# OpenDriveLab/OccNet

Hardware: NVIDIA H100
Metric: samples/s (6-cam->200x200x16 voxel) (higher is better)
Workload: dtype bf16

## Files before the change

include/occ_b200.h:

```cpp
#ifndef OCC_B200_H_
#define OCC_B200_H_

#include <stdint.h>

#ifdef __cplusplus
extern "C" {
#endif

const char* occb200_last_error(void);
const char* occb200_version(void);

int occb200_ms_deform_attn_forward(const float* value, const int64_t* spatial_shapes,
                                   const int64_t* level_start_index, const float* sampling_loc,
                                   const float* attn_weight, int B, int Nv, int M, int C, int Nq, int L, int P,
                                   int im2col_step, float* out, void* stream);

int occb200_ms_deform_attn_backward(const float* value, const int64_t* spatial_shapes, const int64_t* level_start_index,
                                    const float* sampling_loc, const float* attn_weight, const float* grad_output, int B,
                                    int Nv, int M, int C, int Nq, int L, int P, int im2col_step, float* grad_value,
                                    float* grad_sampling_loc, float* grad_attn_weight, void* stream);

typedef struct occb200_engine occb200_engine;
typedef struct occb200_backbone occb200_backbone;

// ... 46 lines not shown
int occb200_engine_forward_video(occb200_engine* e, const float* const* feats, const int32_t* rot_map_dev, int scene_start,
                                 float* bev_embed, float* occ_logits, float* flow, uint8_t* occ_cls_u8, int64_t* occ_cls_i64,
                                 void* stream);
int occb200_engine_submit_host_video(occb200_engine* e, int slot, const float* const* feats_host, const int32_t* rot_map_host,
                                     int scene_start, int64_t* occ_cls_i64_host, float* flow_host, void* stream);
int occb200_engine_forward_video_angle(occb200_engine* e, const float* const* feats, double angle_deg, int scene_start,
                                       float* bev_embed, float* occ_logits, float* flow, uint8_t* occ_cls_u8,
                                       int64_t* occ_cls_i64, void* stream);
int occb200_engine_submit_host_video_angle(occb200_engine* e, int slot, const float* const* feats_host, double angle_deg,
                                           int scene_start, int64_t* occ_cls_i64_host, float* flow_host, void* stream);

int occb200_engine_enable_taps(occb200_engine* e, int enable);
int occb200_engine_copy_tap(occb200_engine* e, int which, int layer, float* dst_dev, void* stream);

int occb200_engine_project_pillars(occb200_engine* e, float* ref_cam, uint8_t* mask, void* stream);
int occb200_engine_launches_per_frame(const occb200_engine* e);
int occb200_engine_profile(occb200_engine* e, int enable);
int occb200_engine_profile_read(occb200_engine* e, float* ms_per_category, int* launches_per_category, int n);

int occb200_render_forward(const float* sigma, const float* origin, const float* points, const float* tindex,
                           int N, int T, int Z, int Y, int X, int64_t M, float* pred_dist, float* gt_dist,
                           float* coord_index, void* stream);

int occb200_ray_metric_accumulate(const uint8_t* sem_pred, const float* flow_pred, const uint8_t* sem_gt,
                                  const float* flow_gt, const void* origins, int origin_is_f64, int T,
                                  const float* rays, int M, double* counters, float* pcd_pred, float* pcd_gt,
                                  void* stream);

int occb200_linear_f32(const float* A, const float* W, const float* bias, const float* residual, float* C, int M,
                       int N, int K, int act, void* stream);
// ... 36 lines not shown
```

occnet_b200/_lib.py:

```python
import ctypes
import os

_HERE = os.path.dirname(os.path.abspath(__file__))
LIB_PATH = os.path.join(_HERE, 'lib', 'libocc_b200.so')

c_f32p = ctypes.c_void_p
_vp = ctypes.c_void_p
_i = ctypes.c_int
_i64 = ctypes.c_int64
_f64 = ctypes.c_double


class OccConfig(ctypes.Structure):
    _fields_ = [('bev_h', _i), ('bev_w', _i), ('embed_dims', _i), ('num_heads', _i), ('num_layers', _i),
                ('num_cams', _i), ('num_levels', _i), ('level_h', _i * 4), ('level_w', _i * 4),
                ('num_points_in_pillar', _i), ('sca_points', _i), ('tsa_points', _i), ('ffn_dim', _i),
                ('pillar_h', _i), ('out_dim', _i), ('num_classes', _i), ('pc_range', ctypes.c_float * 6),
                ('precision', _i), ('use_tensor_cores', _i), ('use_cams_embeds', _i),
                ('rotate_center', _i * 2)]


SIGNATURES = {
    'occb200_last_error': (ctypes.c_char_p, []),
    'occb200_version': (ctypes.c_char_p, []),
# ... 10 lines not shown
    'occb200_engine_set_prev_rotation_angle': (_i, [_vp, _f64]),
    'occb200_rotation_coeffs': (_i, [_f64, _i, _i, _i, _i, _vp]),
    'occb200_engine_rotation_map': (_i, [_vp, _f64, _vp, _vp]),
    'occb200_engine_forward': (_i, [_vp, ctypes.POINTER(_vp), _vp, _vp, _vp, _vp, _vp, _vp, _vp]),
    'occb200_engine_forward_host': (_i, [_vp, ctypes.POINTER(_vp), _vp, _vp, _vp]),
    'occb200_engine_submit_host': (_i, [_vp, _i, ctypes.POINTER(_vp), _vp, _vp, _vp]),
    'occb200_engine_wait_host': (_i, [_vp, _i]),
    'occb200_engine_set_history': (_i, [_vp, _i]),
    'occb200_engine_forward_video': (_i, [_vp, ctypes.POINTER(_vp), _vp, _i, _vp, _vp, _vp, _vp, _vp, _vp]),
    'occb200_engine_submit_host_video': (_i, [_vp, _i, ctypes.POINTER(_vp), _vp, _i, _vp, _vp, _vp]),
    'occb200_engine_forward_video_angle': (_i, [_vp, ctypes.POINTER(_vp), _f64, _i, _vp, _vp, _vp, _vp, _vp, _vp]),
    'occb200_engine_submit_host_video_angle': (_i, [_vp, _i, ctypes.POINTER(_vp), _f64, _i, _vp, _vp, _vp]),
    'occb200_engine_enable_taps': (_i, [_vp, _i]),
    'occb200_engine_copy_tap': (_i, [_vp, _i, _i, _vp, _vp]),
    'occb200_engine_project_pillars': (_i, [_vp, _vp, _vp, _vp]),
    'occb200_engine_launches_per_frame': (_i, [_vp]),
    'occb200_engine_profile': (_i, [_vp, _i]),
    'occb200_engine_profile_read': (_i, [_vp, _vp, _vp, _i]),
    'occb200_render_forward': (_i, [_vp, _vp, _vp, _vp, _i, _i, _i, _i, _i, _i64, _vp, _vp, _vp, _vp]),
    'occb200_ray_metric_accumulate': (_i, [_vp, _vp, _vp, _vp, _vp, _i, _i, _vp, _i, _vp, _vp, _vp, _vp]),
    'occb200_linear_f32': (_i, [_vp, _vp, _vp, _vp, _vp, _i, _i, _i, _i, _vp]),
    'occb200_layernorm_f32': (_i, [_vp, _vp, _vp, _vp, _i, _i, _vp]),
    'occb200_gemm_bf16_tc': (_i, [_vp, _vp, _vp, _vp, _i, _i, _i, _vp]),
    'occb200_gemm_tc': (_i, [_vp, _vp, _i, _vp, _vp, _vp, _vp, _i, _i, _i, _i, _i, _vp]),
    'occb200_gemm_tc_ln': (_i, [_vp, _vp, _vp, _vp, _vp, _vp, _vp, _vp, _vp, _vp, _i, _i, _vp]),
    'occb200_gemm_tc_blocked256': (_i, [_vp, _vp, _vp, _vp, _i, _i, _i, _vp]),
    'occb200_gemm_tc_tsa_inputs': (_i, [_vp, _i, _vp, _vp, _vp, _vp, _vp, _i, _vp, _vp, _vp, _vp, _vp, _i, _i, _i, _vp]),
    'occb200_gemm_tc_split3': (_i, [_vp, _i, _vp, _vp, _vp, _vp, _i, _i, _i, _vp]),
    'occb200_split_bf16': (_i, [_vp, _i, _vp, _i, _i64, _vp, _vp]),
    'occb200_backbone_create': (_vp, [_i, _i, _i, _i, _i]),
# ... 49 lines not shown
```

occnet_b200/csrc/engine.cu:

```cuda
#include <cuda_runtime.h>

#include <algorithm>
#include <cmath>
#include <cstring>
#include <map>
#include <string>
#include <vector>

#include "../../include/occ_b200.h"
#include "common.cuh"
#include "conv3d_tc.cuh"
#include "gemm_tc.cuh"
#include "kernels.cuh"

namespace occ {

static thread_local std::string g_last_error;
void set_last_error(const std::string& msg) { g_last_error = msg; }

namespace {

struct DevBuf {
    void* p = nullptr;
    size_t bytes = 0;
// ... 16 lines not shown
    DevBuf tsa_v_wh, tsa_q_wh, tsa_o_wh, sca_q_wh, sca_v_wh, sca_o_wh, ffn1_wh, ffn2_wh;
    DevBuf tsa_q_wh_fold, tsa_q_const, tsa_q_const_t32;
};

}
}

using namespace occ;

struct occb200_engine {
    occb200_config cfg;
    int Nq = 0, Nv = 0, C = 256;
    LevelGeom lg;
    ScaParams sp;
    bool cameras_set = false, finalized = false, taps = false;
    DevBuf rot_map;
    bool rot_set = false;
    RotGrid rot_grid;
    bool rot_grid_set = false;
    DevBuf hist;
    bool hist_valid = false;
    cudaEvent_t hist_done = nullptr;
    bool hist_recorded = false;
    int feats_bf16 = 0;
    occb200_backbone* bb = nullptr;
    DevBuf bb_levels[4];
    cudaEvent_t bb_free = nullptr;
    bool bb_free_recorded = false;
    std::map<std::string, std::vector<float>> host_params;
    std::vector<LayerW> layers;
// ... 82 lines not shown
    occb200_engine* e; cudaStream_t st; int cat; cudaEvent_t a = nullptr, b = nullptr;
    static cudaEvent_t get(occb200_engine* e) {
        if (e->event_used == e->event_pool.size()) {
            cudaEvent_t ev; cudaEventCreate(&ev); e->event_pool.push_back(ev);
        }
        return e->event_pool[e->event_used++];
    }
    ProfScope(occb200_engine* e_, cudaStream_t st_, int cat_) : e(e_), st(st_), cat(cat_) {
        if (e->profiling) { a = get(e); b = get(e); cudaEventRecord(a, st); }
    }
    ~ProfScope() {
        if (e->profiling) { cudaEventRecord(b, st); e->prof_events.push_back({cat, {a, b}}); }
    }
};

template <typename TA, typename TC>
int gemm(occb200_engine* e, const TA* A, const TA* A2, int K1, const float* W, const void* Wh, const float* bias,
         const float* residual, TC* C, int M, int N, int K, int act, cudaStream_t st)
{
    e->launches++;
    ProfScope ps(e, st, CAT_GEMM);
    if constexpr (sizeof(TA) == 2) {
        if (e->cfg.use_tensor_cores && Wh != nullptr && gemm_tc_supported(M, N, K, A2 != nullptr ? K1 : K)) {
            return gemm_tc<TC>(reinterpret_cast<const bf16*>(A), reinterpret_cast<const bf16*>(A2), K1,
                               reinterpret_cast<const bf16*>(Wh), bias, residual, C, M, N, K, act, st);
        }
    }
    if constexpr (sizeof(TA) == 4 && std::is_same<TC, float>::value) {
        if (e->cfg.use_tensor_cores && e->cfg.precision == 0 && Wh != nullptr && e->split_ws.p != nullptr &&
            gemm_tc_supported(M, N, 3 * K, 2 * K)) {
// ... 144 lines not shown
    const int nq_sca = 8 * c.num_levels * c.sca_points * 3;
    const bool q_half = sizeof(T) == 2 && c.use_tensor_cores && e->layers[0].tsa_q_wh.p != nullptr &&
                        e->layers[0].sca_q_wh.p != nullptr && gemm_tc_supported(Nq, nq_tsa, 2 * C, C) &&
                        gemm_tc_supported(Nq, nq_sca, C, C);
    void* qproj = e->qproj.p;
    T* attn_out = e->attn_out.as<T>();
    const bool hoist_v = sizeof(T) == 2 && c.use_tensor_cores && e->sca_value_all.p != nullptr;
    const bool l0_fold = mode == MODE_FRAME && const_q && !has_prev && e->l0_ready;
    const T* q_t_in = q_t;
    if (hoist_v && mode == MODE_FRAME) {
        e->launches++;
        ProfScope ps(e, st, CAT_GEMM);
        if (gemm_tc_blocked256((const bf16*)tokens, e->sca_v_all_wh.as<bf16>(), e->sca_v_all_b.as<float>(),
                               e->sca_value_all.as<bf16>(), ncam * Nv, c.num_layers * C, C, st)) return 2;
    }
    for (int l = 0; l < c.num_layers; ++l) {
        LayerW& w = e->layers[l];
        const bool fold_pos = fuse_ln && !has_prev && w.tsa_q_wh_fold.p != nullptr && w.tsa_q_const.p != nullptr && q_half;
        if (l == 0 && l0_fold) {
            q_f32 = e->l0_x_f32.as<float>(); x_f32 = e->q_f32.as<float>(); spare_f32 = e->x_f32.as<float>();
            cbuf = q_f32;
            q_t_in = e->l0_q_t.as<T>();
            q_in = q_t; q_pos_in = q_pos_t;
        } else {
            const T* a_v = has_prev ? e->prev_t.as<T>() : q_in;
            T* v_prev = e->tsa_value.as<T>();
            const T* v_cur = has_prev ? e->tsa_v_query.as<T>() + (size_t)l * Nq * C : v_prev;
            const bool tsa_merge = sizeof(T) == 2 && fuse_ln && q_half && w.tsa_v_wh.p != nullptr;
            if (tsa_merge) {
                if constexpr (sizeof(T) == 2) {
// ... 52 lines not shown
            }
        }
        const int rc = q_half ? gemm<T, __half>(e, q_t_in, nullptr, 0, w.sca_q_w.as<float>(), w.sca_q_wh.p, w.sca_q_b.as<float>(),
                                                nullptr, (__half*)qproj, Nq, nq_sca, C, ACT_NONE, st)
                              : gemm<T, float>(e, q_t_in, nullptr, 0, w.sca_q_w.as<float>(), w.sca_q_wh.p, w.sca_q_b.as<float>(),
                                               nullptr, (float*)qproj, Nq, nq_sca, C, ACT_NONE, st);
        if (rc) return 2;
        q_t_in = q_t;
        const T* sca_val = e->sca_value.as<T>();
        if (hoist_v) {
            sca_val = reinterpret_cast<const T*>(e->sca_value_all.as<bf16>() + (size_t)l * ncam * Nv * C);
        } else if (gemm<T, T>(e, tokens, nullptr, 0, w.sca_v_w.as<float>(), w.sca_v_wh.p, w.sca_v_b.as<float>(), nullptr,
                              e->sca_value.as<T>(), ncam * Nv, C, C, ACT_NONE, st)) return 2;
        {
            ProfScope ps(e, st, CAT_SCA);
            if (launch_sca_fused<T>(sca_val, qproj, q_half, e->sp, e->lg, Nv, attn_out, e->hits.as<uint8_t>(), st)) return 2;
        }
        e->launches++;
        if (fuse_ln) {
            if (gemm_ln_fused(e, (const bf16*)attn_out, w.sca_o_wh.p, w.sca_o_b.as<float>(), q_f32, w.ln_g[1].as<float>(),
                              w.ln_b[1].as<float>(), nullptr, x_f32, (bf16*)q_t, nullptr, Nq, C, st)) return 2;
            advance();
        } else {
            if (gemm<T, float>(e, attn_out, nullptr, 0, w.sca_o_w.as<float>(), w.sca_o_wh.p, w.sca_o_b.as<float>(),
                               q_f32, x_f32, Nq, C, C, ACT_NONE, st)) return 2;
            if (e->taps)
                OCC_CUDA(cudaMemcpyAsync(e->tap_sca.as<float>() + (size_t)l * Nq * C, x_f32, (size_t)Nq * C * 4,
                                         cudaMemcpyDeviceToDevice, st));
            {
                ProfScope ps(e, st, CAT_LN);
                if (launch_layernorm<T>(x_f32, w.ln_g[1].as<float>(), w.ln_b[1].as<float>(), nullptr, Nq, C, q_f32, q_t,
// ... 12 lines not shown
                return 2;
            advance();
        } else {
            if (gemm<T, float>(e, e->ffn_h.as<T>(), nullptr, 0, w.ffn2_w.as<float>(), w.ffn2_wh.p, w.ffn2_b.as<float>(),
                               q_f32, x_f32, Nq, C, c.ffn_dim, ACT_NONE, st)) return 2;
            {
                ProfScope ps(e, st, CAT_LN);
                if (launch_layernorm<T>(x_f32, w.ln_g[2].as<float>(), w.ln_b[2].as<float>(), pos, Nq, C, q_f32, y_t,
                                        q_pos_t, st)) return 2;
            }
            e->launches++;
        }
        if (e->taps)
            OCC_CUDA(cudaMemcpyAsync(e->tap_layer.as<float>() + (size_t)l * Nq * C, q_f32, (size_t)Nq * C * 4,
                                     cudaMemcpyDeviceToDevice, st));
    }
    const int X = c.bev_w, Y = c.bev_h, Z = c.pillar_h, mid = C / Z;
    const bool lift_from_t32 = fuse_ln && sizeof(T) == 2 && bev_embed == nullptr && Z == 16 && mid == 16;
    if (fuse_ln && !lift_from_t32) {
        ProfScope ps(e, st, CAT_PACK);
        if (launch_t32_convert(q_f32, x_f32, Nq, 1, st)) return 2;
        advance();
        e->launches++;
    }
    if (bev_embed)
        OCC_CUDA(cudaMemcpyAsync(bev_embed, q_f32, (size_t)Nq * C * 4, cudaMemcpyDeviceToDevice, st));
    if (!occ_logits && !flow && !cls_u8 && !cls_i64) return 0;
    {
        ProfScope ps(e, st, CAT_VOX);
        if (lift_from_t32) {
// ... 214 lines not shown
{
    if (!e) return;
    for (auto& w : e->layers) {
        DevBuf* all[] = {&w.tsa_v_w, &w.tsa_v_b, &w.tsa_q_w, &w.tsa_q_b, &w.tsa_o_w, &w.tsa_o_b, &w.sca_q_w, &w.sca_q_b,
                         &w.sca_v_w, &w.sca_v_b, &w.sca_o_w, &w.sca_o_b, &w.ffn1_w, &w.ffn1_b, &w.ffn2_w, &w.ffn2_b,
                         &w.ln_g[0], &w.ln_g[1], &w.ln_g[2], &w.ln_b[0], &w.ln_b[1], &w.ln_b[2], &w.tsa_v_wh,
                         &w.tsa_q_wh, &w.tsa_o_wh, &w.sca_q_wh, &w.sca_v_wh, &w.sca_o_wh, &w.ffn1_wh, &w.ffn2_wh,
                         &w.tsa_q_wh_fold, &w.tsa_q_const, &w.tsa_q_const_t32};
        for (DevBuf* b : all) b->release();
    }
    DevBuf* all[] = {&e->rot_map, &e->hist, &e->split_ws, &e->tokens_split, &e->l0_x_f32, &e->l0_q_t, &e->pos_bf, &e->qc_f32, &e->qc_t, &e->qc_pos_t, &e->bev_queries, &e->pos, &e->pos_t32, &e->cams_embeds, &e->level_embeds, &e->conv_w[0], &e->conv_w[1],
                     &e->conv_b[0], &e->conv_b[1], &e->conv_wh[0], &e->conv_wh[1], &e->conv_wh_hi[0], &e->conv_wh_hi[1], &e->conv_wh_lo[0],
                     &e->conv_wh_lo[1], &e->vox_split, &e->sca_v_all_wh, &e->sca_v_all_b, &e->sca_value_all, &e->hw1, &e->hb1, &e->hw2, &e->hb2,
                     &e->fw1, &e->fb1, &e->fw2, &e->fb2, &e->head_w1h, &e->head_w2h, &e->head_b1c, &e->head_b2c, &e->tokens, &e->sca_value, &e->q_f32, &e->q_t,
                     &e->q_pos_t, &e->prev_t, &e->tsa_value, &e->tsa_v_query, &e->qproj, &e->attn_out,
                     &e->x_f32, &e->ffn_h, &e->vox0, &e->vox1, &e->vox2, &e->hits, &e->tap_layer, &e->tap_tsa,
                     &e->tap_sca, &e->feats_dev[0], &e->feats_dev[1], &e->feats_dev[2], &e->feats_dev[3],
                     &e->occ_i64_dev, &e->flow_dev, &e->bb_levels[0], &e->bb_levels[1], &e->bb_levels[2], &e->bb_levels[3]};
    for (DevBuf* b : all) b->release();
    if (e->bb_free) cudaEventDestroy(e->bb_free);
    if (e->hist_done) cudaEventDestroy(e->hist_done);
    for (auto& sl : e->slots) {
        for (auto& f : sl.feats) f.release();
        sl.occ.release(); sl.flow.release(); sl.rot.release();
        if (sl.rot_pinned) cudaFreeHost(sl.rot_pinned);
        if (sl.compute_done) {
            for (cudaEvent_t ev : sl.h2d_done) cudaEventDestroy(ev);
            cudaEventDestroy(sl.compute_done); cudaEventDestroy(sl.d2h_done);
        }
    }
    if (e->d2h_stream) {
        for (cudaStream_t hs : e->h2d_stream) cudaStreamDestroy(hs);
        cudaStreamDestroy(e->d2h_stream);
    }
    for (cudaEvent_t ev : e->event_pool) cudaEventDestroy(ev);
    delete e;
// ... 203 lines not shown
                upload(e->head_b1c, b1c.data(), b1c.size()) || upload(e->head_b2c, b2c.data(), b2c.size())) return 2;
        }
    }
    const size_t es = e->elt();
    const size_t nvox = (size_t)c.bev_w * c.bev_h * c.pillar_h;
    const size_t ntok = (size_t)c.num_cams * e->Nv;
    int maxq = 8 * c.num_levels * c.sca_points * 3;
    const size_t nq_pad = ((size_t)Nq + 127) / 128 * 128;
    if (e->tokens.alloc(ntok * C * es) || e->sca_value.alloc(ntok * C * es) || e->q_f32.alloc(nq_pad * C * 4) ||
        e->q_t.alloc((size_t)Nq * C * es) || e->q_pos_t.alloc((size_t)Nq * C * es) ||
        e->prev_t.alloc((size_t)Nq * C * es) || e->tsa_value.alloc((size_t)Nq * C * es) ||
        e->qproj.alloc((size_t)Nq * maxq * 4) ||
        e->attn_out.alloc((size_t)Nq * C * es) || e->x_f32.alloc(nq_pad * C * 4) ||
        e->ffn_h.alloc((size_t)Nq * F * es) || e->vox0.alloc(nvox * mid * es) || e->vox1.alloc(nvox * od * es) ||
        e->vox2.alloc(nvox * od * es) || e->hits.alloc(Nq)) return 2;
    OCC_CUDA(cudaMemset(e->q_f32.p, 0, nq_pad * C * 4));
    OCC_CUDA(cudaMemset(e->x_f32.p, 0, nq_pad * C * 4));
    if (tc32) {
        const size_t kmax = (size_t)std::max(2 * C, F);
        if (e->split_ws.alloc((size_t)Nq * 2 * kmax * 2) || e->tokens_split.alloc(ntok * 2 * C * 2)) return 2;
        if (c.pillar_h == 16 && e->vox_split.alloc(nvox * 2 * od * 2)) return 2;
    }
    e->host_params.clear();
    if ((c.precision == 0 ? build_tsa_query_values<float>(e) : build_tsa_query_values<bf16>(e))) return 2;
    e->l0_ready = false;
    if (tc && e->qc_f32.p != nullptr && getenv("OCC_NO_L0_FOLD") == nullptr) {
        const size_t rows_pad = ((size_t)Nq + 127) / 128 * 128;
        if (e->l0_x_f32.alloc(rows_pad * C * 4) || e->l0_q_t.alloc((size_t)Nq * C * 2)) return 2;
        OCC_CUDA(cudaMemset(e->l0_x_f32.p, 0, rows_pad * C * 4));
        const bool taps = e->taps;
        e->taps = false;
        const int rc = forward_impl<bf16>(e, nullptr, nullptr, nullptr, nullptr, nullptr, nullptr, nullptr, 0, MODE_L0_TSA_ONLY);
        e->taps = taps;
        if (rc) return rc;
        OCC_CUDA(cudaDeviceSynchronize());
        e->l0_ready = true;
    }
    e->finalized = true;
    return 0;
}

int occb200_engine_set_cameras(occb200_engine* e, const float* cam_mat, const float* zs, int img_h, int img_w)
{
    OCC_CHECK(e && cam_mat && zs, "null pointer");
    const occb200_config& c = e->cfg;
    memset(&e->sp, 0, sizeof(e->sp));
    for (int i = 0; i < c.num_cams; ++i)
        for (int k = 0; k < 16; ++k) e->sp.cam_mat[i][k] = cam_mat[i * 16 + k];
    for (int i = 0; i < c.num_points_in_pillar; ++i) e->sp.zs[i] = zs[i];
    for (int i = 0; i < 3; ++i) {
        e->sp.pc_scale[i] = (float)((double)c.pc_range[3 + i] - (double)c.pc_range[i]);
        e->sp.pc_min[i] = c.pc_range[i];
    }
    e->sp.img_w = (float)img_w; e->sp.img_h = (float)img_h;
    e->sp.num_cams = c.num_cams; e->sp.D = c.num_points_in_pillar; e->sp.bev_h = c.bev_h; e->sp.bev_w = c.bev_w;
    e->cameras_set = true;
    return 0;
}

int occb200_engine_forward(occb200_engine* e, const float* const* feats, const float* prev_bev, float* bev_embed,
                           float* occ_logits, float* flow, uint8_t* occ_cls_u8, int64_t* occ_cls_i64, void* stream)
{
    OCC_CHECK(e && feats, "null pointer");
    if (check_frame(e, feats)) return 1;
    return run_frame(e, feats, prev_bev, bev_embed, occ_logits, flow, occ_cls_u8, occ_cls_i64, (cudaStream_t)stream);
}

int occb200_engine_set_history(occb200_engine* e, int enable)
{
    OCC_CHECK(e, "null engine");
    if (e->hist_recorded) OCC_CUDA(cudaEventSynchronize(e->hist_done));
    e->hist_recorded = false;
// ... 266 lines not shown
            OCC_CUDA(cudaMemcpyAsync(dst, e->tokens.p, nt * 4, cudaMemcpyDeviceToDevice, st));
            return 0;
        }
        return launch_bf16_to_f32(e->tokens.as<bf16>(), dst, (int64_t)nt, st);
    }
    set_last_error("unknown tap");
    return 1;
}

int occb200_engine_project_pillars(occb200_engine* e, float* ref_cam, uint8_t* mask, void* stream)
{
    OCC_CHECK(e && ref_cam && mask && e->cameras_set, "null pointer / cameras not set");
    return launch_project_pillars(e->sp, ref_cam, mask, (cudaStream_t)stream);
}

int occb200_engine_launches_per_frame(const occb200_engine* e) { return e ? e->launches : 0; }

int occb200_engine_profile(occb200_engine* e, int enable)
{
    OCC_CHECK(e, "null engine");
    e->profiling = enable != 0;
    e->prof_events.clear();
    e->event_used = 0;
    return 0;
}

int occb200_engine_profile_read(occb200_engine* e, float* ms_per_category, int* launches_per_category, int n)
{
    OCC_CHECK(e && ms_per_category && launches_per_category && n >= CAT_COUNT, "bad arguments");
    OCC_CUDA(cudaDeviceSynchronize());
// ... 122 lines not shown
```

occnet_b200/csrc/kernels.cuh:

```cuda
#pragma once
#include "common.cuh"

typedef struct occb200_backbone occb200_backbone;

namespace occ {

struct ScaParams {
    float cam_mat[8][16];
    float zs[8];
    float pc_scale[3];
    float pc_min[3];
    float img_w, img_h;
    int num_cams, D, bev_h, bev_w;
};

int launch_msda_forward(const float* value, const int64_t* shapes, const int64_t* lstart, const float* loc,
                        const float* wts, int B, int Nv, int M, int C, int Nq, int L, int P, float* out,
                        cudaStream_t stream);
int launch_msda_backward(const float* value, const int64_t* shapes, const int64_t* lstart, const float* loc,
                         const float* wts, const float* grad_out, int B, int Nv, int M, int C, int Nq, int L, int P,
                         float* grad_value, float* grad_loc, float* grad_attn, cudaStream_t stream);
template <typename T>
int launch_tsa_fused(const T* value_prev, const T* value_cur, const void* qproj, bool qproj_is_half, int bev_h, int bev_w,
                     T* out, cudaStream_t stream);
template <typename T>
int launch_sca_fused(const T* value, const void* qproj, bool qproj_is_half, const ScaParams& sp, const LevelGeom& lg, int Nv,
                     T* out, uint8_t* hits, cudaStream_t stream);
int launch_project_pillars(const ScaParams& sp, float* ref_cam, uint8_t* mask, cudaStream_t stream);

template <typename T> int launch_nchw_to_nhwc_small(const float* src, T* dst, int N, int C, int H, int W, cudaStream_t stream);
template <typename T>
int launch_im2col_nhwc(const T* in, T* out, int N, int H, int W, int C, int KH, int KW, int stride, int pad, int Ho, int Wo,
                       int Kpad, cudaStream_t stream);
struct FrameNorm { float mean[3], inv_std[3]; int src_h, src_w, to_rgb; };
template <typename T>
int launch_im2col_frames(const uint8_t* frames, T* out, const FrameNorm& fn, int N, int H, int W, int KH, int KW, int stride,
                         int pad, int Ho, int Wo, int Kpad, cudaStream_t stream);
struct BackboneInfo { int num_images, H, W, precision; bool finalized, frames_set; int src_h, src_w, launches; };
BackboneInfo backbone_info(const occb200_backbone* e);
template <typename T> int launch_maxpool3x3s2_nhwc(const T* in, T* out, int N, int H, int W, int C, int Ho, int Wo, cudaStream_t stream);
template <typename T> int launch_add_relu(const T* a, const T* b, T* out, int64_t n, cudaStream_t stream);
template <typename T>
// ... 57 lines not shown
```

occnet_b200/csrc/msda.cu:

```cuda
#include <cuda_fp16.h>

#include "common.cuh"
#include "kernels.cuh"

namespace occ {

namespace {

template <typename T>
__device__ __forceinline__ void bilinear_acc8(const T* __restrict__ base, int H, int W, int pix_stride,
                                              float h_im, float w_im, float wt, float (&acc)[8])
{
    if (!(h_im > -1.f && w_im > -1.f && h_im < (float)H && w_im < (float)W)) return;
    const int h_lo = (int)floorf(h_im), w_lo = (int)floorf(w_im);
    const float lh = h_im - (float)h_lo, lw = w_im - (float)w_lo;
    const float hh = 1.f - lh, hw = 1.f - lw;
    const bool top = h_lo >= 0, bot = h_lo + 1 <= H - 1, lef = w_lo >= 0, rig = w_lo + 1 <= W - 1;
    const T* p = base + ((int64_t)h_lo * W + w_lo) * pix_stride;
    float v1[8], v2[8], v3[8], v4[8];
    const bool b1 = top && lef, b2 = top && rig, b3 = bot && lef, b4 = bot && rig;
    if (b1) load8(p, v1);
    if (b2) load8(p + pix_stride, v2);
    if (b3) load8(p + (int64_t)W * pix_stride, v3);
    if (b4) load8(p + (int64_t)(W + 1) * pix_stride, v4);
// ... 194 lines not shown
            for (int j = 0; j < 4; ++j) {
                const float2 f = __half22float2(*reinterpret_cast<const __half2*>(&w[j]));
                o[8 * i + 2 * j] = f.x; o[8 * i + 2 * j + 1] = f.y;
            }
        }
    }
}

__device__ __forceinline__ uint4 make_desc(const SamplePrep& sm)
{
    return make_uint4((uint32_t)sm.code, pack_bf16x2(sm.c1, sm.c2), pack_bf16x2(sm.c3, sm.c4), 0u);
}

template <typename QT, int DEPTH, typename GetQ>
__device__ __forceinline__ void sca_pipe_query(GetQ getq, const bf16* __restrict__ value, const QT* __restrict__ qproj,
                                               const ScaParams& sp, const LevelGeom& lg, int Nv, bf16* __restrict__ out,
                                               uint8_t* __restrict__ hits, uint4* dw)
{
    const int lane = threadIdx.x & 31, head = lane >> 2, s = lane & 3;
    const unsigned FULL = 0xffffffffu;

    const float xs = __fdiv_rn((float)(getq() % sp.bev_w) + 0.5f, (float)sp.bev_w);
    const float ys = __fdiv_rn((float)(getq() / sp.bev_w) + 0.5f, (float)sp.bev_h);
    float ru[2], rv[2];
    unsigned vis = 0;
#pragma unroll
    for (int r = 0; r < 2; ++r) {
        const int c = r * 4 + (lane >> 3), z = lane & 7;
        bool ok = false;
        ru[r] = 0.f; rv[r] = 0.f;
        if (c < sp.num_cams && z < sp.D) project_point(sp.cam_mat[c], xs, ys, sp.zs[z], sp, ru[r], rv[r], ok);
        const unsigned b = __ballot_sync(FULL, ok);
#pragma unroll
        for (int k = 0; k < 4; ++k) if ((b >> (8 * k)) & 0xffu) vis |= 1u << (r * 4 + k);
    }
    const int count = __popc(vis);
    if (hits && lane == 0) hits[getq()] = (uint8_t)count;

    float acc[8];
#pragma unroll
    for (int i = 0; i < 8; ++i) acc[i] = 0.f;
    const int own_W = s == 0 ? lg.w[0] : s == 1 ? lg.w[1] : s == 2 ? lg.w[2] : lg.w[3];
    const int own_H = s == 0 ? lg.h[0] : s == 1 ? lg.h[1] : s == 2 ? lg.h[2] : lg.h[3];
    const int own_start = s == 0 ? lg.start[0] : s == 1 ? lg.start[1] : s == 2 ? lg.start[2] : lg.start[3];
    const float own_w = (float)own_W, own_h = (float)own_H;

    for (int c = 0; c < sp.num_cams; ++c) {
        if (!((vis >> c) & 1u)) continue;
        {
            const QT* qp = qproj + (int64_t)getq() * 768;
            float off[16], wl[8];
            load_q<16>(qp + head * 64 + s * 16, off);
            load_q<8>(qp + 512 + head * 32 + s * 8, wl);
            float mx = wl[0];
#pragma unroll
            for (int i = 1; i < 8; ++i) mx = fmaxf(mx, wl[i]);
            mx = fmaxf(mx, __shfl_xor_sync(FULL, mx, 1));
            mx = fmaxf(mx, __shfl_xor_sync(FULL, mx, 2));
            float sum = 0.f;
#pragma unroll
            for (int i = 0; i < 8; ++i) { wl[i] = __expf(wl[i] - mx); sum += wl[i]; }
            sum += __shfl_xor_sync(FULL, sum, 1);
            sum += __shfl_xor_sync(FULL, sum, 2);
            const float inv = __fdividef(1.f, sum);
            const int r = c >> 2;
#pragma unroll
            for (int p = 0; p < 8; ++p) {
                const int asrc = (c & 3) * 8 + (p % sp.D);
                const float u = __shfl_sync(FULL, r ? ru[1] : ru[0], asrc);
                const float v = __shfl_sync(FULL, r ? rv[1] : rv[0], asrc);
                const float w_im = fmaf(u, own_w, off[2 * p] - 0.5f);
                const float h_im = fmaf(v, own_h, off[2 * p + 1] - 0.5f);
                dw[desc_slot(p * 4 + s, head)] = make_desc(prep_sample(h_im, w_im, wl[p] * inv, own_H, own_W, own_start));
            }
        }
        __syncwarp();
        const bf16* vcam = value + ((int64_t)c * Nv * 8 + head) * 32 + s * 8;
        gather_descs<32, DEPTH>(acc, dw, head, [&](int i, const bf16*& base, int& W) { base = vcam; W = lg.w[i & 3]; });
        __syncwarp();
    }
    const float scale = (float)max(count, 1);
#pragma unroll
    for (int i = 0; i < 8; ++i) acc[i] = __fdiv_rn(acc[i], scale);
    store8(out + (int64_t)getq() * 256 + head * 32 + s * 8, acc);
}

template <typename QT, int DEPTH, int MINB, int NW>
__global__ void __launch_bounds__(NW * 32, MINB)
sca_pipe_kernel(const bf16* __restrict__ value, const QT* __restrict__ qproj, ScaParams sp, LevelGeom lg,
                int Nv, bf16* __restrict__ out, uint8_t* __restrict__ hits)
{
    __shared__ uint4 descs[NW][32 * 8];
    auto getq = [] { return (int)(blockIdx.x * NW + (threadIdx.x >> 5)); };
    if (getq() >= sp.bev_h * sp.bev_w) return;
    sca_pipe_query<QT, DEPTH>(getq, value, qproj, sp, lg, Nv, out, hits, descs[threadIdx.x >> 5]);
}

template <int VEC>
__global__ void msda_forward_kernel(const float* __restrict__ value, const int64_t* __restrict__ shapes,
                                    const int64_t* __restrict__ lstart, const float* __restrict__ loc,
                                    const float* __restrict__ wts, int B, int Nv, int M, int C, int Nq,
                                    int L, int P, float* __restrict__ out)
{
    const int slices = C / VEC;
    const int64_t idx = (int64_t)blockIdx.x * blockDim.x + threadIdx.x;
    const int64_t total = (int64_t)B * Nq * M * slices;
    if (idx >= total) return;
    const int s = (int)(idx % slices);
    const int m = (int)((idx / slices) % M);
    const int64_t bq = idx / ((int64_t)slices * M);
// ... 185 lines not shown
                const float v = __shfl_sync(FULL, r ? rv[1] : rv[0], asrc);
                const float w_im = __fadd_rn(u, offn[2 * p]) * own_w - 0.5f;
                const float h_im = __fadd_rn(v, offn[2 * p + 1]) * own_h - 0.5f;
                const SamplePrep sm = prep_sample(h_im, w_im, wl[p], own_H, own_W);
#pragma unroll
                for (int l = 0; l < 4; ++l)
                    shuffle_gather<T>(accu, vcam + (int64_t)lg.start[l] * 256, lg.w[l], sm, grp | l);
            }
        }
    }
    float acc[8];
    accu.finish(acc, (float)max(count, 1), true);
    store8(out + (int64_t)q * 256 + head * 32 + s * 8, acc);
}

}

int launch_msda_forward(const float* value, const int64_t* shapes, const int64_t* lstart, const float* loc,
                        const float* wts, int B, int Nv, int M, int C, int Nq, int L, int P, float* out,
                        cudaStream_t stream)
{
    if ((int64_t)B * Nq == 0) return 0;
    if (C % 8 == 0) {
        const int64_t total = (int64_t)B * Nq * M * (C / 8);
        msda_forward_kernel<8><<<ceil_div(total, 256), 256, 0, stream>>>(value, shapes, lstart, loc, wts, B, Nv, M,
                                                                          C, Nq, L, P, out);
    } else {
        const int64_t total = (int64_t)B * Nq * M * C;
        msda_forward_kernel<1><<<ceil_div(total, 256), 256, 0, stream>>>(value, shapes, lstart, loc, wts, B, Nv, M,
                                                                          C, Nq, L, P, out);
// ... 7 lines not shown
                     cudaStream_t stream)
{
    OCC_CHECK(bev_h >= 2 && bev_w >= 2, "tsa_fused: the BEV grid must be at least 2x2");
    const int Nq = bev_h * bev_w;
    const dim3 grid(ceil_div(Nq, 8));
    if (q_half) tsa_fused_kernel<T, __half><<<grid, 256, 0, stream>>>(value_prev, value_cur, (const __half*)qproj, bev_h, bev_w, out);
    else        tsa_fused_kernel<T, float><<<grid, 256, 0, stream>>>(value_prev, value_cur, (const float*)qproj, bev_h, bev_w, out);
    OCC_CUDA(cudaGetLastError());
    return 0;
}
template int launch_tsa_fused<float>(const float*, const float*, const void*, bool, int, int, float*, cudaStream_t);
template int launch_tsa_fused<bf16>(const bf16*, const bf16*, const void*, bool, int, int, bf16*, cudaStream_t);

template <typename T>
int launch_sca_fused(const T* value, const void* qproj_v, bool q_half, const ScaParams& sp, const LevelGeom& lg, int Nv,
                     T* out, uint8_t* hits, cudaStream_t stream)
{
    OCC_CHECK(lg.num_levels == 4 && sp.num_cams <= 8 && sp.D <= 8 && sp.D >= 1 && 8 % sp.D == 0,
              "sca_fused: supports 4 levels, <= 8 cameras, pillar anchors in {1,2,4,8}");
    for (int l = 0; l < 4; ++l) OCC_CHECK(lg.h[l] >= 2 && lg.w[l] >= 2, "sca_fused: every level must be at least 2x2");
    const int Nq = sp.bev_h * sp.bev_w;
    if constexpr (sizeof(T) == 2) {
        if (q_half) sca_pipe_kernel<__half, 1, 6, 4><<<ceil_div(Nq, 4), 128, 0, stream>>>(value, (const __half*)qproj_v, sp, lg, Nv, out, hits);
        else        sca_pipe_kernel<float, 1, 6, 4><<<ceil_div(Nq, 4), 128, 0, stream>>>(value, (const float*)qproj_v, sp, lg, Nv, out, hits);
    } else {
        OCC_CHECK(!q_half, "sca_fused: the unpipelined kernel reads fp32 projections");
        sca_fused_kernel<T><<<ceil_div(Nq, 8), 256, 0, stream>>>(value, (const float*)qproj_v, sp, lg, Nv, out, hits);
    }
    OCC_CUDA(cudaGetLastError());
    return 0;
}
template int launch_sca_fused<float>(const float*, const void*, bool, const ScaParams&, const LevelGeom&, int, float*,
                                     uint8_t*, cudaStream_t);
template int launch_sca_fused<bf16>(const bf16*, const void*, bool, const ScaParams&, const LevelGeom&, int, bf16*,
                                    uint8_t*, cudaStream_t);

int launch_project_pillars(const ScaParams& sp, float* ref_cam, uint8_t* mask, cudaStream_t stream)
{
    const int64_t total = (int64_t)sp.num_cams * sp.bev_h * sp.bev_w * sp.D;
    project_pillars_kernel<<<ceil_div(total, 256), 256, 0, stream>>>(sp, ref_cam, mask);
    OCC_CUDA(cudaGetLastError());
    return 0;
}

}
```

occnet_b200/engine.py:

```python
import ctypes
import numbers

import numpy as np
import torch

from . import _lib

PRECISIONS = {'fp32': 0, 'bf16': 1}


def _cfg_struct(cfg, precision, use_tensor_cores):
    c = _lib.OccConfig()
    c.bev_h, c.bev_w = cfg['bev_h'], cfg['bev_w']
    c.embed_dims, c.num_heads = cfg['embed_dims'], cfg['num_heads']
    c.num_layers, c.num_cams, c.num_levels = cfg['num_layers'], cfg['num_cams'], cfg['num_levels']
    for i, (h, w) in enumerate(cfg['level_shapes']):
        c.level_h[i], c.level_w[i] = h, w
    c.num_points_in_pillar = cfg['num_points_in_pillar']
    c.sca_points, c.tsa_points = cfg['sca_points'], cfg['tsa_points']
    c.ffn_dim, c.pillar_h, c.out_dim, c.num_classes = cfg['ffn_dim'], cfg['pillar_h'], cfg['out_dim'], cfg['num_classes']
    for i in range(6):
        c.pc_range[i] = cfg['pc_range'][i]
    c.precision = PRECISIONS[precision]
    c.use_tensor_cores = int(use_tensor_cores)
# ... 61 lines not shown
        self.feat_dtype, self.feat_channels_last = dtype, bool(channels_last)

    def attach_backbone(self, backbone):
        with torch.cuda.device(self.device):
            _lib.check(self.lib.occb200_engine_attach_backbone(self._h, None if backbone is None else backbone._h))
        self.backbone = backbone

    def __del__(self):
        h = getattr(self, '_h', None)
        if h is not None and h.value:
            self.lib.occb200_engine_destroy(h)
            self._h = ctypes.c_void_p()

    def set_cameras(self, img_metas):
        cam, zs, h, w = camera_params(self.cfg, img_metas)
        _lib.check(self.lib.occb200_engine_set_cameras(self._h, _lib.ptr(cam), _lib.ptr(zs), h, w))

    def set_prev_rotation(self, index_map):
        if index_map is None:
            _lib.check(self.lib.occb200_engine_set_prev_rotation(self._h, None))
            return
        if isinstance(index_map, numbers.Real):
            _lib.check(self.lib.occb200_engine_set_prev_rotation_angle(self._h, float(index_map)))
            return
        m = np.ascontiguousarray(index_map.cpu().numpy() if isinstance(index_map, torch.Tensor) else index_map, np.int32)
        assert m.shape == (self.Nq,)
        _lib.check(self.lib.occb200_engine_set_prev_rotation(self._h, _lib.ptr(m)))

    def _check_feats(self, feats, cuda):
        if self.feat_dtype == torch.uint8:
            if self.backbone is None:
# ... 177 lines not shown
        else:
            dst = torch.empty((self.Nq, self.cfg['embed_dims']), dtype=torch.float32, device=self.device)
        with torch.cuda.device(self.device):
            _lib.check(self.lib.occb200_engine_copy_tap(self._h, w, layer, _lib.ptr(dst), _lib.stream_ptr()))
        return dst

    def project_pillars(self):
        D = self.cfg['num_points_in_pillar']
        nc = self.cfg['num_cams']
        ref = torch.empty((nc, self.Nq, D, 2), dtype=torch.float32, device=self.device)
        mask = torch.empty((nc, self.Nq, D), dtype=torch.uint8, device=self.device)
        with torch.cuda.device(self.device):
            _lib.check(self.lib.occb200_engine_project_pillars(self._h, _lib.ptr(ref), _lib.ptr(mask), _lib.stream_ptr()))
        return ref, mask

    CATEGORIES = ('pack', 'gemm', 'tsa_gather', 'sca_gather', 'layernorm', 'bev_to_voxel', 'conv3d', 'occ_head')

    def profile(self, on=True):
        _lib.check(self.lib.occb200_engine_profile(self._h, int(on)))

    def profile_read(self):
        ms = np.zeros(8, np.float32)
        n = np.zeros(8, np.int32)
        _lib.check(self.lib.occb200_engine_profile_read(self._h, _lib.ptr(ms), _lib.ptr(n), 8))
        return {c: (float(ms[i]), int(n[i])) for i, c in enumerate(self.CATEGORIES)}

    @property
    def launches_per_frame(self):
        return int(self.lib.occb200_engine_launches_per_frame(self._h))
```

Measured before the change: 209.0.

## Precompute SCA camera projection table once per camera set and tile queries in 2D patches

Moves the per-query camera projection of pillar anchors out of the bf16 SCA gather kernel into a separate geometry kernel. That kernel runs on its own stream only when the camera parameters change, and its results are cached in a uv/mask table. The gather kernel now reads the precomputed anchors and visibility mask instead of recomputing them for every layer. It also maps warps to 4x2 spatial patches of BEV cells for better sampling locality and changes minBlocks and warps per block. The cost is extra device memory, a cross-stream event dependency, and an extra global load per camera, in exchange for removing redundant projection arithmetic.

```diff
diff --git a/include/occ_b200.h b/include/occ_b200.h
--- a/include/occ_b200.h
+++ b/include/occ_b200.h
@@ -84,6 +84,7 @@
 int occb200_engine_copy_tap(occb200_engine* e, int which, int layer, float* dst_dev, void* stream);
 
 int occb200_engine_project_pillars(occb200_engine* e, float* ref_cam, uint8_t* mask, void* stream);
+int occb200_engine_sca_geometry(occb200_engine* e, float* uv, uint8_t* mask, uint8_t* hits, void* stream);
 int occb200_engine_launches_per_frame(const occb200_engine* e);
 int occb200_engine_profile(occb200_engine* e, int enable);
 int occb200_engine_profile_read(occb200_engine* e, float* ms_per_category, int* launches_per_category, int n);
diff --git a/occnet_b200/_lib.py b/occnet_b200/_lib.py
--- a/occnet_b200/_lib.py
+++ b/occnet_b200/_lib.py
@@ -48,6 +48,7 @@
     'occb200_engine_enable_taps': (_i, [_vp, _i]),
     'occb200_engine_copy_tap': (_i, [_vp, _i, _i, _vp, _vp]),
     'occb200_engine_project_pillars': (_i, [_vp, _vp, _vp, _vp]),
+    'occb200_engine_sca_geometry': (_i, [_vp, _vp, _vp, _vp, _vp]),
     'occb200_engine_launches_per_frame': (_i, [_vp]),
     'occb200_engine_profile': (_i, [_vp, _i]),
     'occb200_engine_profile_read': (_i, [_vp, _vp, _vp, _i]),
diff --git a/occnet_b200/csrc/engine.cu b/occnet_b200/csrc/engine.cu
--- a/occnet_b200/csrc/engine.cu
+++ b/occnet_b200/csrc/engine.cu
@@ -54,6 +54,11 @@
     LevelGeom lg;
     ScaParams sp;
     bool cameras_set = false, finalized = false, taps = false;
+    DevBuf geo_uv, geo_mask;
+    bool geo_dirty = true;
+    cudaStream_t geo_stream = nullptr;
+    cudaEvent_t geo_free = nullptr, geo_ready = nullptr;
+    bool geo_free_recorded = false, geo_ready_recorded = false;
     DevBuf rot_map;
     bool rot_set = false;
     RotGrid rot_grid;
@@ -166,6 +171,17 @@
     }
 };
 
+int ensure_sca_geometry(occb200_engine* e)
+{
+    if (!e->geo_dirty || !e->cameras_set || e->geo_uv.p == nullptr) return 0;
+    if (e->geo_free_recorded) OCC_CUDA(cudaStreamWaitEvent(e->geo_stream, e->geo_free, 0));
+    if (launch_sca_geometry(e->sp, e->geo_uv.as<float>(), e->geo_mask.as<uint8_t>(), e->geo_stream)) return 2;
+    OCC_CUDA(cudaEventRecord(e->geo_ready, e->geo_stream));
+    e->geo_ready_recorded = true;
+    e->geo_dirty = false;
+    return 0;
+}
+
 template <typename TA, typename TC>
 int gemm(occb200_engine* e, const TA* A, const TA* A2, int K1, const float* W, const void* Wh, const float* bias,
          const float* residual, TC* C, int M, int N, int K, int act, cudaStream_t st)
@@ -340,6 +356,7 @@
         if (gemm_tc_blocked256((const bf16*)tokens, e->sca_v_all_wh.as<bf16>(), e->sca_v_all_b.as<float>(),
                                e->sca_value_all.as<bf16>(), ncam * Nv, c.num_layers * C, C, st)) return 2;
     }
+    if (sizeof(T) == 2 && mode == MODE_FRAME && e->geo_ready_recorded) OCC_CUDA(cudaStreamWaitEvent(st, e->geo_ready, 0));
     for (int l = 0; l < c.num_layers; ++l) {
         LayerW& w = e->layers[l];
         const bool fold_pos = fuse_ln && !has_prev && w.tsa_q_wh_fold.p != nullptr && w.tsa_q_const.p != nullptr && q_half;
@@ -422,7 +439,8 @@
                               e->sca_value.as<T>(), ncam * Nv, C, C, ACT_NONE, st)) return 2;
         {
             ProfScope ps(e, st, CAT_SCA);
-            if (launch_sca_fused<T>(sca_val, qproj, q_half, e->sp, e->lg, Nv, attn_out, e->hits.as<uint8_t>(), st)) return 2;
+            if (launch_sca_fused<T>(sca_val, qproj, q_half, e->sp, e->lg, Nv, e->geo_uv.as<float>(), e->geo_mask.as<uint8_t>(),
+                                    attn_out, e->hits.as<uint8_t>(), st)) return 2;
         }
         e->launches++;
         if (fuse_ln) {
@@ -465,6 +483,10 @@
         if (e->taps)
             OCC_CUDA(cudaMemcpyAsync(e->tap_layer.as<float>() + (size_t)l * Nq * C, q_f32, (size_t)Nq * C * 4,
                                      cudaMemcpyDeviceToDevice, st));
+    }
+    if (sizeof(T) == 2 && mode == MODE_FRAME) {
+        OCC_CUDA(cudaEventRecord(e->geo_free, st));
+        e->geo_free_recorded = true;
     }
     const int X = c.bev_w, Y = c.bev_h, Z = c.pillar_h, mid = C / Z;
     const bool lift_from_t32 = fuse_ln && sizeof(T) == 2 && bev_embed == nullptr && Z == 16 && mid == 16;
@@ -709,12 +731,16 @@
                      &e->conv_wh_lo[1], &e->vox_split, &e->sca_v_all_wh, &e->sca_v_all_b, &e->sca_value_all, &e->hw1, &e->hb1, &e->hw2, &e->hb2,
                      &e->fw1, &e->fb1, &e->fw2, &e->fb2, &e->head_w1h, &e->head_w2h, &e->head_b1c, &e->head_b2c, &e->tokens, &e->sca_value, &e->q_f32, &e->q_t,
                      &e->q_pos_t, &e->prev_t, &e->tsa_value, &e->tsa_v_query, &e->qproj, &e->attn_out,
-                     &e->x_f32, &e->ffn_h, &e->vox0, &e->vox1, &e->vox2, &e->hits, &e->tap_layer, &e->tap_tsa,
+                     &e->x_f32, &e->ffn_h, &e->vox0, &e->vox1, &e->vox2, &e->hits, &e->geo_uv, &e->geo_mask, &e->tap_layer, &e->tap_tsa,
                      &e->tap_sca, &e->feats_dev[0], &e->feats_dev[1], &e->feats_dev[2], &e->feats_dev[3],
                      &e->occ_i64_dev, &e->flow_dev, &e->bb_levels[0], &e->bb_levels[1], &e->bb_levels[2], &e->bb_levels[3]};
     for (DevBuf* b : all) b->release();
     if (e->bb_free) cudaEventDestroy(e->bb_free);
     if (e->hist_done) cudaEventDestroy(e->hist_done);
+    if (e->geo_stream) {
+        cudaStreamSynchronize(e->geo_stream);
+        cudaStreamDestroy(e->geo_stream); cudaEventDestroy(e->geo_free); cudaEventDestroy(e->geo_ready);
+    }
     for (auto& sl : e->slots) {
         for (auto& f : sl.feats) f.release();
         sl.occ.release(); sl.flow.release(); sl.rot.release();
@@ -948,6 +974,16 @@
         e->attn_out.alloc((size_t)Nq * C * es) || e->x_f32.alloc(nq_pad * C * 4) ||
         e->ffn_h.alloc((size_t)Nq * F * es) || e->vox0.alloc(nvox * mid * es) || e->vox1.alloc(nvox * od * es) ||
         e->vox2.alloc(nvox * od * es) || e->hits.alloc(Nq)) return 2;
+    if (c.precision != 0) {
+        if (e->geo_uv.alloc((size_t)Nq * c.num_cams * 8 * 2 * 4) || e->geo_mask.alloc(Nq)) return 2;
+        if (!e->geo_stream) {
+            OCC_CUDA(cudaStreamCreateWithFlags(&e->geo_stream, cudaStreamNonBlocking));
+            OCC_CUDA(cudaEventCreateWithFlags(&e->geo_free, cudaEventDisableTiming));
+            OCC_CUDA(cudaEventCreateWithFlags(&e->geo_ready, cudaEventDisableTiming));
+        }
+        e->geo_dirty = true;
+        if (ensure_sca_geometry(e)) return 2;
+    }
     OCC_CUDA(cudaMemset(e->q_f32.p, 0, nq_pad * C * 4));
     OCC_CUDA(cudaMemset(e->x_f32.p, 0, nq_pad * C * 4));
     if (tc32) {
@@ -978,18 +1014,22 @@
 {
     OCC_CHECK(e && cam_mat && zs, "null pointer");
     const occb200_config& c = e->cfg;
-    memset(&e->sp, 0, sizeof(e->sp));
+    ScaParams sp;
+    memset(&sp, 0, sizeof(sp));
     for (int i = 0; i < c.num_cams; ++i)
-        for (int k = 0; k < 16; ++k) e->sp.cam_mat[i][k] = cam_mat[i * 16 + k];
-    for (int i = 0; i < c.num_points_in_pillar; ++i) e->sp.zs[i] = zs[i];
+        for (int k = 0; k < 16; ++k) sp.cam_mat[i][k] = cam_mat[i * 16 + k];
+    for (int i = 0; i < c.num_points_in_pillar; ++i) sp.zs[i] = zs[i];
     for (int i = 0; i < 3; ++i) {
-        e->sp.pc_scale[i] = (float)((double)c.pc_range[3 + i] - (double)c.pc_range[i]);
-        e->sp.pc_min[i] = c.pc_range[i];
-    }
-    e->sp.img_w = (float)img_w; e->sp.img_h = (float)img_h;
-    e->sp.num_cams = c.num_cams; e->sp.D = c.num_points_in_pillar; e->sp.bev_h = c.bev_h; e->sp.bev_w = c.bev_w;
+        sp.pc_scale[i] = (float)((double)c.pc_range[3 + i] - (double)c.pc_range[i]);
+        sp.pc_min[i] = c.pc_range[i];
+    }
+    sp.img_w = (float)img_w; sp.img_h = (float)img_h;
+    sp.num_cams = c.num_cams; sp.D = c.num_points_in_pillar; sp.bev_h = c.bev_h; sp.bev_w = c.bev_w;
+    if (e->cameras_set && memcmp(&sp, &e->sp, sizeof(sp)) == 0) return 0;
+    e->sp = sp;
+    e->geo_dirty = true;
     e->cameras_set = true;
-    return 0;
+    return ensure_sca_geometry(e);
 }
 
 int occb200_engine_forward(occb200_engine* e, const float* const* feats, const float* prev_bev, float* bev_embed,
@@ -1286,6 +1326,17 @@
     return launch_project_pillars(e->sp, ref_cam, mask, (cudaStream_t)stream);
 }
 
+int occb200_engine_sca_geometry(occb200_engine* e, float* uv, uint8_t* mask, uint8_t* hits, void* stream)
+{
+    OCC_CHECK(e && e->cameras_set && e->finalized && e->cfg.precision != 0, "bf16 engine not finalized / cameras not set");
+    cudaStream_t st = (cudaStream_t)stream;
+    if (e->geo_ready_recorded) OCC_CUDA(cudaStreamWaitEvent(st, e->geo_ready, 0));
+    if (uv) OCC_CUDA(cudaMemcpyAsync(uv, e->geo_uv.p, e->geo_uv.bytes, cudaMemcpyDeviceToDevice, st));
+    if (mask) OCC_CUDA(cudaMemcpyAsync(mask, e->geo_mask.p, e->geo_mask.bytes, cudaMemcpyDeviceToDevice, st));
+    if (hits) OCC_CUDA(cudaMemcpyAsync(hits, e->hits.p, e->hits.bytes, cudaMemcpyDeviceToDevice, st));
+    return 0;
+}
+
 int occb200_engine_launches_per_frame(const occb200_engine* e) { return e ? e->launches : 0; }
 
 int occb200_engine_profile(occb200_engine* e, int enable)
diff --git a/occnet_b200/csrc/kernels.cuh b/occnet_b200/csrc/kernels.cuh
--- a/occnet_b200/csrc/kernels.cuh
+++ b/occnet_b200/csrc/kernels.cuh
@@ -25,7 +25,8 @@
                      T* out, cudaStream_t stream);
 template <typename T>
 int launch_sca_fused(const T* value, const void* qproj, bool qproj_is_half, const ScaParams& sp, const LevelGeom& lg, int Nv,
-                     T* out, uint8_t* hits, cudaStream_t stream);
+                     const float* geo_uv, const uint8_t* geo_mask, T* out, uint8_t* hits, cudaStream_t stream);
+int launch_sca_geometry(const ScaParams& sp, float* uv, uint8_t* mask, cudaStream_t stream);
 int launch_project_pillars(const ScaParams& sp, float* ref_cam, uint8_t* mask, cudaStream_t stream);
 
 template <typename T> int launch_nchw_to_nhwc_small(const float* src, T* dst, int N, int C, int H, int W, cudaStream_t stream);
diff --git a/occnet_b200/csrc/msda.cu b/occnet_b200/csrc/msda.cu
--- a/occnet_b200/csrc/msda.cu
+++ b/occnet_b200/csrc/msda.cu
@@ -232,26 +232,14 @@
 
 template <typename QT, int DEPTH, typename GetQ>
 __device__ __forceinline__ void sca_pipe_query(GetQ getq, const bf16* __restrict__ value, const QT* __restrict__ qproj,
-                                               const ScaParams& sp, const LevelGeom& lg, int Nv, bf16* __restrict__ out,
+                                               const float2* __restrict__ geo_uv, const uint8_t* __restrict__ geo_mask,
+                                               int num_cams, const LevelGeom& lg, int Nv, bf16* __restrict__ out,
                                                uint8_t* __restrict__ hits, uint4* dw)
 {
     const int lane = threadIdx.x & 31, head = lane >> 2, s = lane & 3;
     const unsigned FULL = 0xffffffffu;
 
-    const float xs = __fdiv_rn((float)(getq() % sp.bev_w) + 0.5f, (float)sp.bev_w);
-    const float ys = __fdiv_rn((float)(getq() / sp.bev_w) + 0.5f, (float)sp.bev_h);
-    float ru[2], rv[2];
-    unsigned vis = 0;
-#pragma unroll
-    for (int r = 0; r < 2; ++r) {
-        const int c = r * 4 + (lane >> 3), z = lane & 7;
-        bool ok = false;
-        ru[r] = 0.f; rv[r] = 0.f;
-        if (c < sp.num_cams && z < sp.D) project_point(sp.cam_mat[c], xs, ys, sp.zs[z], sp, ru[r], rv[r], ok);
-        const unsigned b = __ballot_sync(FULL, ok);
-#pragma unroll
-        for (int k = 0; k < 4; ++k) if ((b >> (8 * k)) & 0xffu) vis |= 1u << (r * 4 + k);
-    }
+    const unsigned vis = __ldg(geo_mask + getq());
     const int count = __popc(vis);
     if (hits && lane == 0) hits[getq()] = (uint8_t)count;
 
@@ -263,9 +251,10 @@
     const int own_start = s == 0 ? lg.start[0] : s == 1 ? lg.start[1] : s == 2 ? lg.start[2] : lg.start[3];
     const float own_w = (float)own_W, own_h = (float)own_H;
 
-    for (int c = 0; c < sp.num_cams; ++c) {
+    for (int c = 0; c < num_cams; ++c) {
         if (!((vis >> c) & 1u)) continue;
         {
+            const float2 anchor = __ldg(geo_uv + ((int64_t)getq() * num_cams + c) * 8 + (lane & 7));
             const QT* qp = qproj + (int64_t)getq() * 768;
             float off[16], wl[8];
             load_q<16>(qp + head * 64 + s * 16, off);
@@ -281,12 +270,10 @@
             sum += __shfl_xor_sync(FULL, sum, 1);
             sum += __shfl_xor_sync(FULL, sum, 2);
             const float inv = __fdividef(1.f, sum);
-            const int r = c >> 2;
 #pragma unroll
             for (int p = 0; p < 8; ++p) {
-                const int asrc = (c & 3) * 8 + (p % sp.D);
-                const float u = __shfl_sync(FULL, r ? ru[1] : ru[0], asrc);
-                const float v = __shfl_sync(FULL, r ? rv[1] : rv[0], asrc);
+                const float u = __shfl_sync(FULL, anchor.x, p);
+                const float v = __shfl_sync(FULL, anchor.y, p);
                 const float w_im = fmaf(u, own_w, off[2 * p] - 0.5f);
                 const float h_im = fmaf(v, own_h, off[2 * p + 1] - 0.5f);
                 dw[desc_slot(p * 4 + s, head)] = make_desc(prep_sample(h_im, w_im, wl[p] * inv, own_H, own_W, own_start));
@@ -303,15 +290,50 @@
     store8(out + (int64_t)getq() * 256 + head * 32 + s * 8, acc);
 }
 
-template <typename QT, int DEPTH, int MINB, int NW>
+template <int NW, int PW>
+__device__ __forceinline__ int sca_query_of(int b, int w, int bev_h, int bev_w)
+{
+    constexpr int PH = NW / PW;
+    const int tiles_x = (bev_w + PW - 1) / PW;
+    const int x = (b % tiles_x) * PW + w % PW, y = (b / tiles_x) * PH + w / PW;
+    return x < bev_w && y < bev_h ? y * bev_w + x : -1;
+}
+
+template <typename QT, int DEPTH, int MINB, int NW, int PW>
 __global__ void __launch_bounds__(NW * 32, MINB)
-sca_pipe_kernel(const bf16* __restrict__ value, const QT* __restrict__ qproj, ScaParams sp, LevelGeom lg,
-                int Nv, bf16* __restrict__ out, uint8_t* __restrict__ hits)
-{
+sca_pipe_kernel(const bf16* __restrict__ value, const QT* __restrict__ qproj, const float2* __restrict__ geo_uv,
+                const uint8_t* __restrict__ geo_mask, int num_cams, int bev_h, int bev_w, LevelGeom lg, int Nv,
+                bf16* __restrict__ out, uint8_t* __restrict__ hits)
+{
+    static_assert(NW % PW == 0, "a patch is PW cells wide");
     __shared__ uint4 descs[NW][32 * 8];
-    auto getq = [] { return (int)(blockIdx.x * NW + (threadIdx.x >> 5)); };
-    if (getq() >= sp.bev_h * sp.bev_w) return;
-    sca_pipe_query<QT, DEPTH>(getq, value, qproj, sp, lg, Nv, out, hits, descs[threadIdx.x >> 5]);
+    auto getq = [=] { return sca_query_of<NW, PW>((int)blockIdx.x, (int)(threadIdx.x >> 5), bev_h, bev_w); };
+    if (getq() < 0) return;
+    sca_pipe_query<QT, DEPTH>(getq, value, qproj, geo_uv, geo_mask, num_cams, lg, Nv, out, hits, descs[threadIdx.x >> 5]);
+}
+
+__global__ void sca_geometry_kernel(ScaParams sp, float2* __restrict__ uv, uint8_t* __restrict__ mask)
+{
+    const int q = (int)((blockIdx.x * blockDim.x + threadIdx.x) >> 5);
+    if (q >= sp.bev_h * sp.bev_w) return;
+    const int lane = threadIdx.x & 31, p = lane & 7;
+    const float xs = __fdiv_rn((float)(q % sp.bev_w) + 0.5f, (float)sp.bev_w);
+    const float ys = __fdiv_rn((float)(q / sp.bev_w) + 0.5f, (float)sp.bev_h);
+    unsigned vis = 0;
+#pragma unroll
+    for (int r = 0; r < 2; ++r) {
+        const int c = r * 4 + (lane >> 3);
+        float u = 0.f, v = 0.f;
+        bool ok = false;
+        if (c < sp.num_cams) {
+            project_point(sp.cam_mat[c], xs, ys, sp.zs[p % sp.D], sp, u, v, ok);
+            uv[((int64_t)q * sp.num_cams + c) * 8 + p] = make_float2(u, v);
+        }
+        const unsigned b = __ballot_sync(0xffffffffu, ok);
+#pragma unroll
+        for (int k = 0; k < 4; ++k) if ((b >> (8 * k)) & 0xffu) vis |= 1u << (r * 4 + k);
+    }
+    if (lane == 0) mask[q] = (uint8_t)vis;
 }
 
 template <int VEC>
@@ -527,6 +549,8 @@
     store8(out + (int64_t)q * 256 + head * 32 + s * 8, acc);
 }
 
+constexpr int SCA_DEPTH = 1, SCA_MINB = 3, SCA_NW = 8, SCA_PW = 4;
+
 }
 
 int launch_msda_forward(const float* value, const int64_t* shapes, const int64_t* lstart, const float* loc,
@@ -564,15 +588,20 @@
 
 template <typename T>
 int launch_sca_fused(const T* value, const void* qproj_v, bool q_half, const ScaParams& sp, const LevelGeom& lg, int Nv,
-                     T* out, uint8_t* hits, cudaStream_t stream)
+                     const float* geo_uv, const uint8_t* geo_mask, T* out, uint8_t* hits, cudaStream_t stream)
 {
     OCC_CHECK(lg.num_levels == 4 && sp.num_cams <= 8 && sp.D <= 8 && sp.D >= 1 && 8 % sp.D == 0,
               "sca_fused: supports 4 levels, <= 8 cameras, pillar anchors in {1,2,4,8}");
     for (int l = 0; l < 4; ++l) OCC_CHECK(lg.h[l] >= 2 && lg.w[l] >= 2, "sca_fused: every level must be at least 2x2");
     const int Nq = sp.bev_h * sp.bev_w;
     if constexpr (sizeof(T) == 2) {
-        if (q_half) sca_pipe_kernel<__half, 1, 6, 4><<<ceil_div(Nq, 4), 128, 0, stream>>>(value, (const __half*)qproj_v, sp, lg, Nv, out, hits);
-        else        sca_pipe_kernel<float, 1, 6, 4><<<ceil_div(Nq, 4), 128, 0, stream>>>(value, (const float*)qproj_v, sp, lg, Nv, out, hits);
+        OCC_CHECK(geo_uv != nullptr && geo_mask != nullptr, "sca_fused: the bf16 gather needs the camera geometry table");
+        const int grid = ceil_div(sp.bev_w, SCA_PW) * ceil_div(sp.bev_h, SCA_NW / SCA_PW);
+        const float2* uv = reinterpret_cast<const float2*>(geo_uv);
+        if (q_half) sca_pipe_kernel<__half, SCA_DEPTH, SCA_MINB, SCA_NW, SCA_PW><<<grid, SCA_NW * 32, 0, stream>>>(
+                        value, (const __half*)qproj_v, uv, geo_mask, sp.num_cams, sp.bev_h, sp.bev_w, lg, Nv, out, hits);
+        else        sca_pipe_kernel<float, SCA_DEPTH, SCA_MINB, SCA_NW, SCA_PW><<<grid, SCA_NW * 32, 0, stream>>>(
+                        value, (const float*)qproj_v, uv, geo_mask, sp.num_cams, sp.bev_h, sp.bev_w, lg, Nv, out, hits);
     } else {
         OCC_CHECK(!q_half, "sca_fused: the unpipelined kernel reads fp32 projections");
         sca_fused_kernel<T><<<ceil_div(Nq, 8), 256, 0, stream>>>(value, (const float*)qproj_v, sp, lg, Nv, out, hits);
@@ -580,10 +609,18 @@
     OCC_CUDA(cudaGetLastError());
     return 0;
 }
-template int launch_sca_fused<float>(const float*, const void*, bool, const ScaParams&, const LevelGeom&, int, float*,
-                                     uint8_t*, cudaStream_t);
-template int launch_sca_fused<bf16>(const bf16*, const void*, bool, const ScaParams&, const LevelGeom&, int, bf16*,
-                                    uint8_t*, cudaStream_t);
+template int launch_sca_fused<float>(const float*, const void*, bool, const ScaParams&, const LevelGeom&, int, const float*,
+                                     const uint8_t*, float*, uint8_t*, cudaStream_t);
+template int launch_sca_fused<bf16>(const bf16*, const void*, bool, const ScaParams&, const LevelGeom&, int, const float*,
+                                    const uint8_t*, bf16*, uint8_t*, cudaStream_t);
+
+int launch_sca_geometry(const ScaParams& sp, float* uv, uint8_t* mask, cudaStream_t stream)
+{
+    OCC_CHECK(sp.num_cams <= 8 && sp.D >= 1 && sp.D <= 8, "sca_geometry: <= 8 cameras, 1..8 pillar anchors");
+    sca_geometry_kernel<<<ceil_div(sp.bev_h * sp.bev_w, 8), 256, 0, stream>>>(sp, reinterpret_cast<float2*>(uv), mask);
+    OCC_CUDA(cudaGetLastError());
+    return 0;
+}
 
 int launch_project_pillars(const ScaParams& sp, float* ref_cam, uint8_t* mask, cudaStream_t stream)
 {
diff --git a/occnet_b200/engine.py b/occnet_b200/engine.py
--- a/occnet_b200/engine.py
+++ b/occnet_b200/engine.py
@@ -99,7 +99,8 @@
 
     def set_cameras(self, img_metas):
         cam, zs, h, w = camera_params(self.cfg, img_metas)
-        _lib.check(self.lib.occb200_engine_set_cameras(self._h, _lib.ptr(cam), _lib.ptr(zs), h, w))
+        with torch.cuda.device(self.device):
+            _lib.check(self.lib.occb200_engine_set_cameras(self._h, _lib.ptr(cam), _lib.ptr(zs), h, w))
 
     def set_prev_rotation(self, index_map):
         if index_map is None:
@@ -307,6 +308,16 @@
             _lib.check(self.lib.occb200_engine_project_pillars(self._h, _lib.ptr(ref), _lib.ptr(mask), _lib.stream_ptr()))
         return ref, mask
 
+    def sca_geometry(self):
+        nc = self.cfg['num_cams']
+        uv = torch.empty((self.Nq, nc, 8, 2), dtype=torch.float32, device=self.device)
+        mask = torch.empty((self.Nq,), dtype=torch.uint8, device=self.device)
+        hits = torch.empty((self.Nq,), dtype=torch.uint8, device=self.device)
+        with torch.cuda.device(self.device):
+            _lib.check(self.lib.occb200_engine_sca_geometry(self._h, _lib.ptr(uv), _lib.ptr(mask), _lib.ptr(hits),
+                                                            _lib.stream_ptr()))
+        return uv, mask, hits
+
     CATEGORIES = ('pack', 'gemm', 'tsa_gather', 'sca_gather', 'layernorm', 'bev_to_voxel', 'conv3d', 'occ_head')
 
     def profile(self, on=True):
```

Result: faster. 214.9 (median of 6 runs) (+2.8%).
